# choice17/ransac_with_homography

Hardware: AMD Instinct MI355X
Metric: backward-warp Mpixels/sec (+ RANSAC hypotheses/sec) (higher is better)
Workload: dtype u8 (f64 coordinates, f32 blend); 1 GPU; transformImageH warp 3840x2160 RGB u8 bilinear -> 2028x3771 u8, 32 distinct frames per GPU per step, Hs mild perspective; full=False

## Files before the change

### ransac_with_homography_amd/csrc/rwh_warp_rgb8.h

```cpp
#pragma once
#include "rwh_common.h"
#include <type_traits>

namespace rwh {

typedef float f2 __attribute__((ext_vector_type(2)));

constexpr double MAGIC = 1572864.0;
constexpr uint32_t MAGIC_HI = 0x41380000u;
constexpr unsigned long long MAGIC_BITS = 0x4138000000000000ull;
constexpr float W_SCALE = 5.42101086242752217e-20f;
constexpr float U8_BIAS = -0.5f + 3.0517578125e-05f;

constexpr int FP_PX = 4;
constexpr int FP_ROWS = 9;
constexpr int FP_LANES = 21;
constexpr int FP_TEXELS = 4 * FP_LANES;
constexpr int FP_PITCH = 4 * FP_TEXELS + 16;

struct Coef {
    double cx[3], cy[3], cw[3];
    double dxs8[7][3];
    double ih[9];
    long long image;
// ... 840 lines not shown
            __builtin_amdgcn_fence(__ATOMIC_ACQUIRE, "wavefront");
        }
        const uint32_t bx = MAGIC_HI + (uint32_t)wxmn, by = MAGIC_HI + (uint32_t)wymn;
        const uint32_t rx_max = (uint32_t)(4 * wC - 2), ry_max = (uint32_t)(wnrows - 2);
#pragma unroll
        for (int h = 0; h < 2; ++h) {
            unsigned vbits = 0u;
            run_coords(h);
#pragma unroll
            for (int j = 0; j < FP_PX; ++j) {
                const bool valid = pixel_valid(j);
                weights2(lx[j], ly[j], valid ? WS : 0.f, valid ? WO : 0.f, valid ? WC : 0.f, wx0[j], wx1[j], wy0[j], wy1[j]);
                vbits |= (unsigned)valid << j;
                const uint32_t rx = min(hx[j] - bx, rx_max), ry = min(hy[j] - by, ry_max);
                const uint32_t lo = mad24_s(ry, (uint32_t)Win::LPITCH, rx << 2);
                const uint32_t* t0 = reinterpret_cast<const uint32_t*>(my + lo);
                const uint32_t* t1 = reinterpret_cast<const uint32_t*>(my + lo + Win::LPITCH);
                a0[j] = t0[0]; b0[j] = t0[1]; a1[j] = t1[0]; b1[j] = t1[1];
            }
            finish_masked_run(h, vbits);
        }
        return;
    }

    unsigned todo = 3u;
    if constexpr (HALVES) {
        todo = wpos ? 0u : 3u;
        if (wpos) {
            constexpr uint32_t lpitch = Win::LPITCH;
            chunk_t vh[2][Win::PASSES];
            int hrows[2];
            uint32_t tapc[2];
            bool hact[2];
#pragma unroll
            for (int h = 0; h < 2; ++h) {
                run_coords(h);
                const uint32_t lhx = h == 0 ? ehx[0] : hx[0], lhy = h == 0 ? ehy[0] : hy[0];
                const uint32_t rhx = h == 0 ? hx[3] : ehx[1], rhy = h == 0 ? hy[3] : ehy[1];
                const int hx0 = (int)__builtin_amdgcn_readlane(lhx, 0), hx1 = (int)__builtin_amdgcn_readlane(rhx, LPR - 1);
                const int hx2 = (int)__builtin_amdgcn_readlane(lhx, 64 - LPR), hx3 = (int)__builtin_amdgcn_readlane(rhx, 63);
                const int hy0 = (int)__builtin_amdgcn_readlane(lhy, 0), hy1 = (int)__builtin_amdgcn_readlane(rhy, LPR - 1);
                const int hy2 = (int)__builtin_amdgcn_readlane(lhy, 64 - LPR), hy3 = (int)__builtin_amdgcn_readlane(rhy, 63);
                const int qxmn = smin(smin(hx0, hx1), smin(hx2, hx3)) & ~3, qxmx = smax(smax(hx0, hx1), smax(hx2, hx3));
                const int qymn = smin(smin(hy0, hy1), smin(hy2, hy3)), qymx = smax(smax(hy0, hy1), smax(hy2, hy3));
                const int sxmn = (int)((uint32_t)smax(qxmn, 0) - MAGIC_HI), sxmx = (int)((uint32_t)smax(qxmx, 0) - MAGIC_HI);
                const int symn = (int)((uint32_t)smax(qymn, 0) - MAGIC_HI), symx = (int)((uint32_t)smax(qymx, 0) - MAGIC_HI);
                const int nr = symx - symn + 2, hC = (sxmx - sxmn + 5) >> 2;
                const bool hfits = (sxmn >= 0) & (sxmx < a.bound_w - 1) & (symn >= 0) & (symx < min(a.bound_h - 1, a.src_h - 2)) &
                                   (nr >= Win::RPP) & (nr <= Win::ROWS) & (hC <= Win::LPRW);
                hrows[h] = hfits ? nr : 0;
                hact[h] = (srow < Win::RPP) & (scol < hC);
                tapc[h] = ((uint32_t)qymn & 0xFFFFFFu) * lpitch + ((uint32_t)qxmn << 2) - slab_off_w;
                if (hfits) {
                    const unsigned char* gbase = simg + (size_t)((uint32_t)symn * pitch + (uint32_t)sxmn * (uint32_t)CH);
#pragma unroll
                    for (int p = 0; p < Win::PASSES; ++p)
                        if (p * Win::RPP < nr && hact[h])
                            __builtin_memcpy(&vh[h][p], gbase + (size_t)((uint32_t)min(p * Win::RPP, nr - Win::RPP) * pitch) + goff, sizeof(chunk_t));
                } else {
                    todo |= 1u << h;
                }
            }
#pragma unroll
            for (int h = 0; h < 2; ++h) {
                if (hrows[h] == 0) continue;
#pragma unroll
                for (int p = 0; p < Win::PASSES; ++p)
                    if (p * Win::RPP < hrows[h] && hact[h]) {
                        uint4 t4;
                        if constexpr (CH == 4) {
                            t4.x = vh[h][p].a; t4.y = vh[h][p].b; t4.z = vh[h][p].c; t4.w = vh[h][p].d;
                        } else {
                            t4.x = vh[h][p].a & 0xFFFFFFu;
                            t4.y = __builtin_amdgcn_perm(vh[h][p].b, vh[h][p].a, 0x0C050403u);
                            t4.z = __builtin_amdgcn_perm(vh[h][p].c, vh[h][p].b, 0x0C040302u);
                            t4.w = vh[h][p].c >> 8;
                        }
                        *reinterpret_cast<uint4*>(my + (uint32_t)min(p * Win::RPP, hrows[h] - Win::RPP) * lpitch + wl) = t4;
                    }
                __builtin_amdgcn_fence(__ATOMIC_RELEASE, "wavefront");
                __builtin_amdgcn_wave_barrier();
                __builtin_amdgcn_fence(__ATOMIC_ACQUIRE, "wavefront");
                if (h == 0) run_coords(0);
#pragma unroll
                for (int j = 0; j < FP_PX; ++j) {
                    weights2(lx[j], ly[j], WS, WO, WC, wx0[j], wx1[j], wy0[j], wy1[j]);
                    const uint32_t lo = mad24_s(hy[j], lpitch, shl2_add_s(hx[j], 0u - tapc[h]));
                    const uint32_t* t0 = reinterpret_cast<const uint32_t*>(slab0 + lo);
                    const uint32_t* t1 = reinterpret_cast<const uint32_t*>(slab0 + lo + lpitch);
                    a0[j] = t0[0]; b0[j] = t0[1]; a1[j] = t1[0]; b1[j] = t1[1];
                }
                const int first = tshift - (lcol + (PW / 2) * h);
                blend_store<DstT, PSTR, CH, true>(a0, b0, a1, b1, wx0, wx1, wy0, wy1, drow + CH * (PW / 2) * h,
                                                  store_any & (first <= 3 * PSTR), max(first, 0));
                __builtin_amdgcn_fence(__ATOMIC_RELEASE, "wavefront");
                __builtin_amdgcn_wave_barrier();
                if (h == 0 && hrows[1] != 0) run_coords(1);
            }
        }
        if (todo == 0u) return;
    }

#pragma unroll
    for (int h = 0; h < 2; ++h) {
        uint32_t off[FP_PX];
        bool near_end = false;
        unsigned vbits = 0u;
        if (HALVES && !(todo & (1u << h))) continue;
        run_coords(h);
#pragma unroll
        for (int j = 0; j < FP_PX; ++j) {
            const bool valid = pixel_valid(j);
            const int ix = (int)(hx[j] - MAGIC_HI), iy = (int)(hy[j] - MAGIC_HI);
            weights2(lx[j], ly[j], valid ? WS : 0.f, valid ? WO : 0.f, valid ? WC : 0.f, wx0[j], wx1[j], wy0[j], wy1[j]);
            off[j] = valid ? (uint32_t)iy * pitch + (uint32_t)ix * (uint32_t)CH : 0u;
            near_end |= valid & (iy > a.src_h - 3);
            vbits |= (unsigned)valid << j;
        }
        if (!__any(vbits != 0u)) {
#pragma unroll
            for (int j = 0; j < FP_PX; ++j) { a0[j] = 0u; b0[j] = 0u; a1[j] = 0u; b1[j] = 0u; }
        } else if (!__any(near_end)) {
#pragma unroll
            for (int j = 0; j < FP_PX; ++j) {
                const pk2 r0 = ld8(simg + off[j]);
                const pk2 r1 = ld8(simg + off[j] + pitch);
                if constexpr (CH == 4) { a0[j] = r0.a; b0[j] = r0.b; a1[j] = r1.a; b1[j] = r1.b; }
                else {
                    a0[j] = r0.a & 0xFFFFFFu; b0[j] = __builtin_amdgcn_perm(r0.b, r0.a, 0x0C050403u);
                    a1[j] = r1.a & 0xFFFFFFu; b1[j] = __builtin_amdgcn_perm(r1.b, r1.a, 0x0C050403u);
                }
            }
        } else {
            const uint32_t last = (uint32_t)a.src_h * pitch - (uint32_t)CH;
#pragma unroll
            for (int j = 0; j < FP_PX; ++j) {
                const uint32_t o00 = off[j];
                const uint32_t o01 = min(o00 + (uint32_t)CH, last), o10 = min(o00 + pitch, last), o11 = min(o00 + pitch + (uint32_t)CH, last);
                if constexpr (CH == 4) {
                    a0[j] = ld4(simg + o00); b0[j] = ld4(simg + o01); a1[j] = ld4(simg + o10); b1[j] = ld4(simg + o11);
                    continue;
                }
                a0[j] = simg[o00] | (simg[o00 + 1] << 8) | (simg[o00 + 2] << 16);
                b0[j] = simg[o01] | (simg[o01 + 1] << 8) | (simg[o01 + 2] << 16);
                a1[j] = simg[o10] | (simg[o10 + 1] << 8) | (simg[o10 + 2] << 16);
                b1[j] = simg[o11] | (simg[o11 + 1] << 8) | (simg[o11 + 2] << 16);
                if constexpr (EXT_SLAB) __builtin_amdgcn_sched_barrier(0);
            }
        }
        finish_masked_run(h, vbits);
    }
}

constexpr int F8_WALK_WAVES = 5;
template <int LOG_PW> __device__ __forceinline__ void fast8mb_body(const FastArgs& a);
template <typename DstT, int LOG_PW, bool WALK = false>
__global__ __launch_bounds__(256, (WALK ? F8_WALK_WAVES : f8_waves<DstT, LOG_PW>())) void warp_rgb8_fast8(const FastArgs a) {
    if constexpr (WALK) {
        static_assert(sizeof(DstT) == 1, "the batch form is uint8 in, uint8 out");
        fast8mb_body<LOG_PW>(a);
    } else {
        fast8_body<DstT, LOG_PW>(a, nullptr);
    }
}
#ifndef RWH_F8H_WAVES
#define RWH_F8H_WAVES(log_pw) ((log_pw) == 5 ? 4 : 5)
#endif
template <int LOG_PW>
__global__ __launch_bounds__(256, RWH_F8H_WAVES(LOG_PW)) void warp_rgb8_fast8h(const FastArgs a) { fast8_body<unsigned char, LOG_PW, false, 3, true>(a, nullptr); }
template <int LOG_PW>
__global__ __launch_bounds__(256, RWH_F8H_WAVES(LOG_PW)) void warp_rgb8_fast8h_tab(const FastArgs a, const CoefTab t) { fast8_body<unsigned char, LOG_PW, false, 3, true>(a, t.e); }
template <int LOG_PW>
__global__ __launch_bounds__(256, 6) void warp_rgba8_fast8(const FastArgs a) { fast8_body<unsigned char, LOG_PW, false, 4>(a, nullptr); }
template <int LOG_PW>
__global__ __launch_bounds__(256, 6) void warp_rgb8_comp(const FastArgs a, const CompArgs c) { fast8_body<unsigned char, LOG_PW, true>(a, nullptr, &c); }
template <typename DstT, int LOG_PW>
__global__ __launch_bounds__(256, (f8_waves<DstT, LOG_PW>())) void warp_rgb8_fast8_tab(const FastArgs a, const CoefTab t) { fast8_body<DstT, LOG_PW>(a, t.e); }

__device__ __forceinline__ pk3 pack_run_u8(const float (&o)[FP_PX][3]) {
    pk3 w;
    uint32_t q = 0;
    q = __builtin_amdgcn_cvt_pk_u8_f32(o[0][0], 0, q); q = __builtin_amdgcn_cvt_pk_u8_f32(o[0][1], 1, q);
    q = __builtin_amdgcn_cvt_pk_u8_f32(o[0][2], 2, q); q = __builtin_amdgcn_cvt_pk_u8_f32(o[1][0], 3, q);
    w.a = q; q = 0;
    q = __builtin_amdgcn_cvt_pk_u8_f32(o[1][1], 0, q); q = __builtin_amdgcn_cvt_pk_u8_f32(o[1][2], 1, q);
    q = __builtin_amdgcn_cvt_pk_u8_f32(o[2][0], 2, q); q = __builtin_amdgcn_cvt_pk_u8_f32(o[2][1], 3, q);
    w.b = q; q = 0;
    q = __builtin_amdgcn_cvt_pk_u8_f32(o[2][2], 0, q); q = __builtin_amdgcn_cvt_pk_u8_f32(o[3][0], 1, q);
    q = __builtin_amdgcn_cvt_pk_u8_f32(o[3][1], 2, q); q = __builtin_amdgcn_cvt_pk_u8_f32(o[3][2], 3, q);
    w.c = q;
    return w;
}
__device__ __forceinline__ void store_run_pk(const pk3& w, unsigned char* drow, bool store_any, int shift) {
    if (!store_any) return;
#ifdef RWH_F8M_STORE_MOD
    if (shift == 0) {
        typedef uint32_t u3s __attribute__((ext_vector_type(3)));
        const u3s d = {w.a, w.b, w.c};
        asm volatile("global_store_dwordx3 %0, %1, off " RWH_F8M_STORE_MOD "\n\ts_nop 2" : : "v"(drow), "v"(d) : "memory");
        return;
    }
#else
    if (shift == 0) { __builtin_memcpy(drow, &w, 12); return; }
#endif
    const unsigned long long lo8 = ((unsigned long long)w.b << 32) | w.a;
#pragma unroll
    for (int i = 3; i < 12; ++i)
        if (i >= 3 * shift) drow[i] = (unsigned char)(i < 8 ? lo8 >> (8 * i) : w.c >> (8 * (i - 8)));
}
#ifndef RWH_F8M_SKEW
#define RWH_F8M_SKEW 8
#endif
__device__ __forceinline__ void store_run_u8(const float (&o)[FP_PX][3], unsigned char* drow, bool store_any, int shift) {
    if (!store_any) return;
    if (shift == 0) {
        pk3 w;
        uint32_t q = 0;
        q = __builtin_amdgcn_cvt_pk_u8_f32(o[0][0], 0, q); q = __builtin_amdgcn_cvt_pk_u8_f32(o[0][1], 1, q);
        q = __builtin_amdgcn_cvt_pk_u8_f32(o[0][2], 2, q); q = __builtin_amdgcn_cvt_pk_u8_f32(o[1][0], 3, q);
        w.a = q; q = 0;
        q = __builtin_amdgcn_cvt_pk_u8_f32(o[1][1], 0, q); q = __builtin_amdgcn_cvt_pk_u8_f32(o[1][2], 1, q);
        q = __builtin_amdgcn_cvt_pk_u8_f32(o[2][0], 2, q); q = __builtin_amdgcn_cvt_pk_u8_f32(o[2][1], 3, q);
        w.b = q; q = 0;
        q = __builtin_amdgcn_cvt_pk_u8_f32(o[2][2], 0, q); q = __builtin_amdgcn_cvt_pk_u8_f32(o[3][0], 1, q);
        q = __builtin_amdgcn_cvt_pk_u8_f32(o[3][1], 2, q); q = __builtin_amdgcn_cvt_pk_u8_f32(o[3][2], 3, q);
        w.c = q;
        __builtin_memcpy(drow, &w, 12);
    } else {
#pragma unroll
        for (int j = 1; j < FP_PX; ++j)
            if (j >= shift) {
#pragma unroll
                for (int k = 0; k < 3; ++k) drow[3 * j + k] = (unsigned char)__builtin_amdgcn_cvt_pk_u8_f32(o[j][k], 0, 0);
            }
    }
}

template <int LOG_PW>
__device__ __forceinline__ void fast8m_body(const FastArgs& a) {
    constexpr int PW = 1 << LOG_PW, PH = 512 / PW, LPR = PW / 8, WX = 128 / PW;
    using Win = F8Window<LOG_PW>;
    constexpr uint32_t lpitch = Win::LPITCH + RWH_F8M_SKEW;
    constexpr int SLAB = ((Win::ROWS * (int)lpitch + 15) / 16) * 16;
    static_assert(SLAB >= Win::SLAB, "the per-frame fallback body shares this slab");
    constexpr float WS = W_SCALE * MIX_S, WO = W_ONE * MIX_S, WC = MIX_S;
    static_assert(MIX_RGB, "the multi-frame kernel is written for the float16-halves blend");
    unsigned char* const slab0 = wave_slabs<SLAB>();

    const unsigned b = blockIdx.x;
    const unsigned logical = (b & 7u) * a.mf_cpx + (b >> 3);
    if (logical >= a.mf_nblocks) return;
    const unsigned g = a.ntiles_magic ? __umulhi(logical, a.ntiles_magic) : (a.ntiles == 1u ? logical : 0u);
    const unsigned ti = logical - g * a.ntiles;
    const int f0 = (int)g * a.mf_frames, f1 = min(f0 + a.mf_frames, a.mf_batch);
    const unsigned ty = a.tiles_x_magic ? __umulhi(ti, a.tiles_x_magic) : ti;
    const unsigned tx = ti - ty * a.tiles_x;
    const int wave = __builtin_amdgcn_readfirstlane((int)(threadIdx.x >> 6));
    const int pwave = wave;
    {
        const int own_from = (int)tx * 128 - min((int)tx * 128, a.out_w - 128);
        if ((wave % WX + 1) * PW <= own_from) return;
    }
    const Coef& co = a.c;
    const int lane = threadIdx.x & 63;
    const int prow = lane / LPR, pq = lane % LPR;
    const int wave_x = (wave % WX) * PW, wave_y = (wave / WX) * PH;
    const int rr_raw = (int)ty * 16 + wave_y + prow;
    const int rr = min(rr_raw, a.rows - 1);
    const int tcol0 = (int)tx * 128;
    const int tcol = min(tcol0, a.out_w - 128);
    const int tshift = tcol0 - tcol;
    const int lcol = wave_x + pq * 4;
    const int c0p = tcol + lcol;
    const bool store_any = rr_raw < a.rows;
    const uint32_t pitch = (uint32_t)a.src_w * 3u;

    const double fr = (double)(a.row_begin + rr), fc = (double)c0p;
    const double X0 = fma(fc, co.cx[2], fma(fr, co.cx[1], co.cx[0]));
    const double Y0 = fma(fc, co.cy[2], fma(fr, co.cy[1], co.cy[0]));
    const double W0 = fma(fc, co.cw[2], fma(fr, co.cw[1], co.cw[0]));
    uint32_t ehx[2], ehy[2], elx[2], ely[2];
    bool wpos;
    {
        const double X7 = X0 + co.dxs8[6][0], Y7 = Y0 + co.dxs8[6][1], W7 = W0 + co.dxs8[6][2];
        double r0 = __builtin_amdgcn_rcp(W0); r0 = fma(fma(-W0, r0, 1.0), r0, r0);
        double r7 = __builtin_amdgcn_rcp(W7); r7 = fma(fma(-W7, r7, 1.0), r7, r7);
        const double ux0 = fma(X0, r0, MAGIC), uy0 = fma(Y0, r0, MAGIC), ux7 = fma(X7, r7, MAGIC), uy7 = fma(Y7, r7, MAGIC);
        ehx[0] = hi32(ux0); elx[0] = lo32(ux0); ehy[0] = hi32(uy0); ely[0] = lo32(uy0);
        ehx[1] = hi32(ux7); elx[1] = lo32(ux7); ehy[1] = hi32(uy7); ely[1] = lo32(uy7);
        const int h0 = (int)hi32(W0), h7 = (int)hi32(W7);
        wpos = __all((int)(h0 > 0x2D300000) & (int)(h0 < 0x52B00000) & (int)(h7 > 0x2D300000) & (int)(h7 < 0x52B00000));
    }
    const int x0 = (int)__builtin_amdgcn_readlane(ehx[0], 0), x1 = (int)__builtin_amdgcn_readlane(ehx[1], LPR - 1);
    const int x2 = (int)__builtin_amdgcn_readlane(ehx[0], 64 - LPR), x3 = (int)__builtin_amdgcn_readlane(ehx[1], 63);
    const int y0 = (int)__builtin_amdgcn_readlane(ehy[0], 0), y1 = (int)__builtin_amdgcn_readlane(ehy[1], LPR - 1);
    const int y2 = (int)__builtin_amdgcn_readlane(ehy[0], 64 - LPR), y3 = (int)__builtin_amdgcn_readlane(ehy[1], 63);
    const int hxmn = smin(smin(x0, x1), smin(x2, x3)) & ~3, hxmx = smax(smax(x0, x1), smax(x2, x3));
    const int hymn = smin(smin(y0, y1), smin(y2, y3)), hymx = smax(smax(y0, y1), smax(y2, y3));
    const int xmn = (int)((uint32_t)smax(hxmn, 0) - MAGIC_HI), xmx = (int)((uint32_t)smax(hxmx, 0) - MAGIC_HI);
    const int ymn = (int)((uint32_t)smax(hymn, 0) - MAGIC_HI), ymx = (int)((uint32_t)smax(hymx, 0) - MAGIC_HI);
    const int nrows = ymx - ymn + 2, C = (xmx - xmn + 5) >> 2;
    const bool staged = wpos & (xmn >= 0) & (xmx < a.bound_w - 1) & (ymn >= 0) & (ymx < min(a.bound_h - 1, a.src_h - 2)) &
                        (nrows >= Win::RPP) & (nrows <= Win::ROWS) & (C <= Win::LPRW);
    if (!staged) {
        for (int f = f0; f < f1; ++f)
            fast8_body<unsigned char, LOG_PW, false, 3, false, true>(a, nullptr, nullptr, (int)((unsigned)f * a.ntiles + ti), slab0 + pwave * SLAB);
        return;
// ... 26 lines not shown
#else
            asm volatile("s_mov_b64 %1, exec\n\ts_mov_b64 exec, %4\n\tglobal_load_dwordx3 %0, %2, %3\n\ts_mov_b64 exec, %1"
                         : "=&v"(v[p]), "=&s"(keep) : "v"(goff), "s"(rowbase), "s"(m) : "memory");
#endif
#endif
        }
    };
    auto landed = [&](u3 (&v)[Win::PASSES]) __attribute__((always_inline)) {
        if constexpr (Win::PASSES == 5) asm volatile("s_waitcnt vmcnt(0)" : "+v"(v[0]), "+v"(v[1]), "+v"(v[2]), "+v"(v[3]), "+v"(v[4]) : : "memory");
        else {
#pragma unroll
            for (int p = 0; p < Win::PASSES; ++p) asm volatile("s_waitcnt vmcnt(0)" : "+v"(v[p]) : : "memory");
        }
    };
    auto expand = [&](const u3 (&v)[Win::PASSES]) __attribute__((always_inline)) {
#pragma unroll
        for (int p = 0; p < Win::PASSES; ++p)
            if (p * Win::RPP < nrows && sactive) {
                const int r0 = min(p * Win::RPP, nrows - Win::RPP);
                uint4 t4;
                t4.x = v[p].x & 0xFFFFFFu;
                t4.y = __builtin_amdgcn_perm(v[p].y, v[p].x, 0x0C050403u);
                t4.z = __builtin_amdgcn_perm(v[p].z, v[p].y, 0x0C040302u);
                t4.w = v[p].z >> 8;
                __builtin_memcpy(__builtin_assume_aligned(my + (uint32_t)r0 * lpitch + wl, RWH_F8M_SKEW % 16 ? 8 : 16), &t4, 16);
            }
        __builtin_amdgcn_fence(__ATOMIC_RELEASE, "wavefront");
        __builtin_amdgcn_wave_barrier();
        __builtin_amdgcn_fence(__ATOMIC_ACQUIRE, "wavefront");
    };
    u3 v[Win::PASSES], v1[Win::PASSES];
#ifdef RWH_F8M_EARLY1
    issue(gsrc, v1);
#ifdef RWH_F8M_EARLY2
    if (f0 + 1 < f1) issue(gsrc + a.src_img_stride, v);
#endif
#endif

    const uint32_t slab_off = (uint32_t)pwave * (uint32_t)SLAB;
    const uint32_t tap_c = ((uint32_t)hymn & 0xFFFFFFu) * lpitch + ((uint32_t)hxmn << 2) - slab_off;
    float wa[F8_PX], wb[F8_PX], wc[F8_PX], wd[F8_PX];
    uint32_t lo[F8_PX];
#pragma unroll
    for (int h = 0; h < 2; ++h) {
        double X[3], Y[3], W[3], rc[3];
        uint32_t lx[FP_PX], ly[FP_PX], hx[FP_PX], hy[FP_PX];
#pragma unroll
        for (int j = 0; j < 3; ++j) { X[j] = X0 + co.dxs8[3 * h + j][0]; Y[j] = Y0 + co.dxs8[3 * h + j][1]; W[j] = W0 + co.dxs8[3 * h + j][2]; }
        const double p12 = W[0] * W[1], P = p12 * W[2];
        double rp = __builtin_amdgcn_rcp(P);
        rp = fma(fma(-P, rp, 1.0), rp, rp);
        const double r12 = rp * W[2];
        rc[2] = rp * p12; rc[0] = r12 * W[1]; rc[1] = r12 * W[0];
#pragma unroll
        for (int j = 0; j < 3; ++j) {
            const double ux = fma(X[j], rc[j], MAGIC), uy = fma(Y[j], rc[j], MAGIC);
            const int q = j + 1 - h;
            hx[q] = hi32(ux); lx[q] = lo32(ux); hy[q] = hi32(uy); ly[q] = lo32(uy);
        }
        hx[3 * h] = ehx[h]; lx[3 * h] = elx[h]; hy[3 * h] = ehy[h]; ly[3 * h] = ely[h];
#pragma unroll
        for (int j = 0; j < FP_PX; ++j) {
            const int p = 4 * h + j;
            const float wx1 = (float)lx[j], wy1 = (float)ly[j] * WS;
            const float w11 = wx1 * wy1;
            const float w01 = __builtin_fmaf(wx1, WO, -w11);
            const float w10 = __builtin_fmaf(wy1, 4294967296.0f, -w11);
            const float w00 = __builtin_fmaf(-wx1, WO, WC) - w10;
            wa[p] = w00; wb[p] = w01; wc[p] = w10; wd[p] = w11;
            lo[p] = mad24_s(hy[j], lpitch, shl2_add_s(hx[j], 0u - tap_c));
        }
    }

#ifdef RWH_F8M_EARLY1
#pragma unroll
    for (int p = 0; p < F8_PX; ++p) asm volatile("" : : "v"(wa[p]), "v"(wb[p]), "v"(wc[p]), "v"(wd[p]), "v"(lo[p]));
#else
    issue(gsrc, v1);
#endif
    landed(v1);
    expand(v1);
#ifndef RWH_F8M_EARLY2
    if (f0 + 1 < f1) issue(gsrc + a.src_img_stride, v);
#endif
#ifdef RWH_LAB_STAMPS
    unsigned long long tA = 0, tB = 0, tC = 0, tD = 0, t0 = __builtin_amdgcn_s_memtime(), t1;
#define RWH_STAMP(acc) { t1 = __builtin_amdgcn_s_memtime(); acc += t1 - t0; t0 = t1; }
#else
#define RWH_STAMP(acc)
#endif
    for (int f = f0; f < f1; ++f) {
        gsrc += a.src_img_stride;
        const bool more = f + 1 < f1;
        pk3 w[2];
#pragma unroll
        for (int h = 0; h < 2; ++h) {
            float o[FP_PX][3];
#pragma unroll
            for (int j = 0; j < FP_PX; ++j) {
                const int p = 4 * h + j;
                const uint32_t* t0 = reinterpret_cast<const uint32_t*>(slab0 + lo[p]);
                const uint32_t* t1 = reinterpret_cast<const uint32_t*>(slab0 + lo[p] + lpitch);
                const uint32_t a0 = t0[0], b0 = t0[1], a1 = t1[0], b1 = t1[1];
                const float w00 = wa[p], w01 = wb[p], w10 = wc[p], w11 = wd[p];
                const uint32_t g00 = rg_halves(a0), g01 = rg_halves(b0), g10 = rg_halves(a1), g11 = rg_halves(b1);
                o[j][0] = fmix_lo(g11, w11, fmix_lo(g10, w10, fmix_lo(g01, w01, fmix_lo_c(g00, w00, U8_BIAS))));
                o[j][1] = fmix_hi(g11, w11, fmix_hi(g10, w10, fmix_hi(g01, w01, fmix_hi_c(g00, w00, U8_BIAS))));
                o[j][2] = fmix_hi(b1, w11, fmix_hi(a1, w10, fmix_hi(b0, w01, fmix_hi_c(a0, w00, U8_BIAS))));
            }
            w[h] = pack_run_u8(o);
        }
        __builtin_amdgcn_fence(__ATOMIC_RELEASE, "wavefront");
        __builtin_amdgcn_wave_barrier();
        RWH_STAMP(tA)
        if (more) { landed(v); RWH_STAMP(tB) expand(v); }
        RWH_STAMP(tC)
        unsigned char* drow = gdst + doff;
#pragma unroll
        for (int h = 0; h < 2; ++h) {
            const int first = tshift - (lcol + (PW / 2) * h);
#ifdef RWH_ABL_M_NOSTORE
            if (w[h].a + w[h].b == 0x12345u)
#endif
            store_run_pk(w[h], drow + 3 * (PW / 2) * h, store_any & (first <= 3), max(first, 0));
        }
        gdst += a.dst_img_stride;
        if (f + 2 < f1) issue(gsrc + a.src_img_stride, v);
        RWH_STAMP(tD)
    }
#ifdef RWH_LAB_STAMPS
    if (lane == 0 && logical < 8192u) {
        unsigned long long* st = reinterpret_cast<unsigned long long*>(a.dst) + ((size_t)logical * 4 + pwave) * 4;
        st[0] = tA; st[1] = tB; st[2] = tC; st[3] = tD;
    }
#endif
}
constexpr int BCH = 36, BROWS = 21;
__device__ __forceinline__ void lds_barrier() { asm volatile("s_waitcnt lgkmcnt(0)\n\ts_barrier" : : : "memory"); }
__device__ __forceinline__ const FastArgs& kernarg_fastargs() {
    typedef const FastArgs __attribute__((address_space(4))) kFastArgs;
    kFastArgs* p = (kFastArgs*)__builtin_amdgcn_kernarg_segment_ptr();
    asm volatile("" : "+s"(p));
    return *(const FastArgs*)p;
}
template <int LOG_PW>
__device__ __forceinline__ void fast8mb_body(const FastArgs& a) {
    constexpr int PW = 1 << LOG_PW, PH = 512 / PW, LPR = PW / 8, WX = 128 / PW;
    using Win = F8Window<LOG_PW>;
    constexpr uint32_t lpitch = BCH * 16 + RWH_F8M_SKEW;
    constexpr int SLABW = ((Win::ROWS * (int)(Win::LPITCH + RWH_F8M_SKEW) + 15) / 16) * 16;
    static_assert(4 * SLABW >= BROWS * (int)lpitch + 128, "the block window lives in the four waves' slabs");
    constexpr float WS = W_SCALE * MIX_S, WO = W_ONE * MIX_S, WC = MIX_S;
    unsigned char* const slab0 = wave_slabs<SLABW>();

    const unsigned b = blockIdx.x;
    const unsigned logical = (b & 7u) * a.mf_cpx + (b >> 3);
    if (logical >= a.mf_nblocks) return;
    const unsigned g = a.ntiles_magic ? __umulhi(logical, a.ntiles_magic) : (a.ntiles == 1u ? logical : 0u);
    const unsigned ti = logical - g * a.ntiles;
    const int f0 = (int)g * a.mf_frames, f1 = min(f0 + a.mf_frames, a.mf_batch);
    const unsigned ty = a.tiles_x_magic ? __umulhi(ti, a.tiles_x_magic) : ti;
    const unsigned tx = ti - ty * a.tiles_x;
    const int wave = __builtin_amdgcn_readfirstlane((int)(threadIdx.x >> 6));
    const Coef& co = a.c;
    const int lane = threadIdx.x & 63;
    const int prow = lane / LPR, pq = lane % LPR;
    const int wave_x = (wave % WX) * PW, wave_y = (wave / WX) * PH;
    const int rr_raw = (int)ty * 16 + wave_y + prow;
    const int rr = min(rr_raw, a.rows - 1);
    const int tcol0 = (int)tx * 128;
    const int tcol = min(tcol0, a.out_w - 128);
    const int tshift = tcol0 - tcol;
    const int lcol = wave_x + pq * 4;
    const int c0p = tcol + lcol;
    const bool store_any = rr_raw < a.rows;
    const uint32_t pitch = (uint32_t)a.src_w * 3u;

    const double fr = (double)(a.row_begin + rr), fc = (double)c0p;
    const double X0 = fma(fc, co.cx[2], fma(fr, co.cx[1], co.cx[0]));
    const double Y0 = fma(fc, co.cy[2], fma(fr, co.cy[1], co.cy[0]));
    const double W0 = fma(fc, co.cw[2], fma(fr, co.cw[1], co.cw[0]));
    uint32_t ehx[2], ehy[2], elx[2], ely[2];
    bool wpos;
    {
        const double X7 = X0 + co.dxs8[6][0], Y7 = Y0 + co.dxs8[6][1], W7 = W0 + co.dxs8[6][2];
        double r0 = __builtin_amdgcn_rcp(W0); r0 = fma(fma(-W0, r0, 1.0), r0, r0);
        double r7 = __builtin_amdgcn_rcp(W7); r7 = fma(fma(-W7, r7, 1.0), r7, r7);
        const double ux0 = fma(X0, r0, MAGIC), uy0 = fma(Y0, r0, MAGIC), ux7 = fma(X7, r7, MAGIC), uy7 = fma(Y7, r7, MAGIC);
        ehx[0] = hi32(ux0); elx[0] = lo32(ux0); ehy[0] = hi32(uy0); ely[0] = lo32(uy0);
        ehx[1] = hi32(ux7); elx[1] = lo32(ux7); ehy[1] = hi32(uy7); ely[1] = lo32(uy7);
        const int h0 = (int)hi32(W0), h7 = (int)hi32(W7);
        wpos = __all((int)(h0 > 0x2D300000) & (int)(h0 < 0x52B00000) & (int)(h7 > 0x2D300000) & (int)(h7 < 0x52B00000));
    }
    const int x0 = (int)__builtin_amdgcn_readlane(ehx[0], 0), x1 = (int)__builtin_amdgcn_readlane(ehx[1], LPR - 1);
    const int x2 = (int)__builtin_amdgcn_readlane(ehx[0], 64 - LPR), x3 = (int)__builtin_amdgcn_readlane(ehx[1], 63);
    const int y0 = (int)__builtin_amdgcn_readlane(ehy[0], 0), y1 = (int)__builtin_amdgcn_readlane(ehy[1], LPR - 1);
    const int y2 = (int)__builtin_amdgcn_readlane(ehy[0], 64 - LPR), y3 = (int)__builtin_amdgcn_readlane(ehy[1], 63);
    const int whxmn = smin(smin(x0, x1), smin(x2, x3)) & ~3, whxmx = smax(smax(x0, x1), smax(x2, x3));
    const int whymn = smin(smin(y0, y1), smin(y2, y3)), whymx = smax(smax(y0, y1), smax(y2, y3));
    const bool owns = (wave % WX + 1) * PW > tshift;
    bool in;
    {
        const int bxmn = (int)((uint32_t)smax(whxmn, 0) - MAGIC_HI), bxmx = (int)((uint32_t)smax(whxmx, 0) - MAGIC_HI);
        const int bymn = (int)((uint32_t)smax(whymn, 0) - MAGIC_HI), bymx = (int)((uint32_t)smax(whymx, 0) - MAGIC_HI);
        const bool outside = wpos & ((bxmx < 0) | (bxmn >= a.bound_w) | (bymx < 0) | (bymn >= a.bound_h));
        const bool interior = wpos & (bxmn >= 0) & (bxmx < a.bound_w - 1) & (bymn >= 0) & (bymx < min(a.bound_h - 1, a.src_h - 2));
        in = owns & !outside;
        const int bw1 = __builtin_amdgcn_readfirstlane(a.bound_w) - 1, bh1 = __builtin_amdgcn_readfirstlane(a.bound_h) - 1;
        int* red = reinterpret_cast<int*>(slab0);
        if (lane == 0) {
            red[5 * wave] = in ? smin(smax(bxmn, 0), bw1) : 0x7FFFFFFF; red[5 * wave + 1] = in ? smin(smax(bxmx, 0), bw1) : -0x7FFFFFFF - 1;
            red[5 * wave + 2] = in ? smin(smax(bymn, 0), bh1) : 0x7FFFFFFF; red[5 * wave + 3] = in ? smin(smax(bymx, 0), bh1) : -0x7FFFFFFF - 1;
            red[5 * wave + 4] = (wpos ? 1 : 0) | ((interior | !owns) ? 2 : 0);
        }
    }
    __syncthreads();
    int xmn, xmx, ymn, ymx, fl_and;
    {
        const int* red = reinterpret_cast<const int*>(slab0);
        xmn = min(min(red[0], red[5]), min(red[10], red[15])); xmx = max(max(red[1], red[6]), max(red[11], red[16]));
        ymn = min(min(red[2], red[7]), min(red[12], red[17])); ymx = max(max(red[3], red[8]), max(red[13], red[18]));
        fl_and = red[4] & red[9] & red[14] & red[19];
        xmn = __builtin_amdgcn_readfirstlane(xmn) & ~3; xmx = __builtin_amdgcn_readfirstlane(xmx);
        ymn = __builtin_amdgcn_readfirstlane(ymn); ymx = __builtin_amdgcn_readfirstlane(ymx);
        fl_and = __builtin_amdgcn_readfirstlane(fl_and);
    }
    __syncthreads();
    const bool any_in = ymn != 0x7FFFFFFF;
    const int nrows = any_in ? ymx - ymn + 2 : 0, C = any_in ? (xmx - xmn + 5) >> 2 : 0;
    const uint32_t doff = ((uint32_t)rr * (uint32_t)a.pitch_w + (uint32_t)c0p) * 3u;
    const bool masked = !(fl_and & 2);
    if (!(fl_and & 1) || (any_in && !(nrows <= BROWS && C <= BCH && ymn + nrows - 1 <= a.src_h - 2))) {
        if (!owns) return;
        for (int f = f0; f < f1; ++f) {
            const FastArgs& ka = kernarg_fastargs();
            fast8_body<unsigned char, LOG_PW, false, 3, false, true>(ka, nullptr, nullptr, (int)((unsigned)f * ka.ntiles + ti), slab0 + wave * SLABW);
        }
        return;
    }
    if (!any_in) {
        if (!owns) return;
        unsigned char* drow = a.dst + (long long)f0 * a.dst_img_stride + doff;
        for (int f = f0; f < f1; ++f) {
#pragma unroll
            for (int h = 0; h < 2; ++h) {
                const int first = tshift - (lcol + (PW / 2) * h);
                zero_store<unsigned char, 1, 3>(drow + 3 * (PW / 2) * h, store_any & (first <= 3), max(first, 0));
            }
            drow += a.dst_img_stride;
        }
        return;
    }

    constexpr int SLOTS = (BROWS * BCH + 255) / 256;
    uint32_t goff[SLOTS], wl[SLOTS];
    unsigned long long smask[SLOTS];
    bool sact[SLOTS];
#pragma unroll
    for (int p = 0; p < SLOTS; ++p) {
        const int c = (int)threadIdx.x + 256 * p, r = c / BCH, k = c - r * BCH;
        sact[p] = (r < nrows) & (k < C);
        goff[p] = mad24_s((uint32_t)r, pitch, mul24_12((uint32_t)k));
        wl[p] = (uint32_t)r * lpitch + (uint32_t)k * 16u;
        smask[p] = __ballot(sact[p]);
    }
    const unsigned char* gsrc = a.src + (long long)f0 * a.src_img_stride + (size_t)((uint32_t)ymn * pitch + (uint32_t)xmn * 3u);
    unsigned char* gdst = a.dst + (long long)f0 * a.dst_img_stride;
    typedef uint32_t u3 __attribute__((ext_vector_type(3)));
    auto issue = [&](const unsigned char* gb, u3 (&v)[SLOTS]) __attribute__((always_inline)) {
#pragma unroll
        for (int p = 0; p < SLOTS; ++p) {
            unsigned long long keep;
            asm volatile("s_mov_b64 %1, exec\n\ts_mov_b64 exec, %4\n\tglobal_load_dwordx3 %0, %2, %3\n\ts_mov_b64 exec, %1"
                         : "=&v"(v[p]), "=&s"(keep) : "v"(goff[p]), "s"(gb), "s"(smask[p]) : "memory");
        }
    };
    auto landed = [&](u3 (&v)[SLOTS]) __attribute__((always_inline)) {
        static_assert(SLOTS == 3, "operand list below");
        asm volatile("s_waitcnt vmcnt(0)" : "+v"(v[0]), "+v"(v[1]), "+v"(v[2]) : : "memory");
    };
    auto expand = [&](const u3 (&v)[SLOTS]) __attribute__((always_inline)) {
#pragma unroll
        for (int p = 0; p < SLOTS; ++p)
            if (sact[p]) {
                uint4 t4;
                t4.x = v[p].x & 0xFFFFFFu;
                t4.y = __builtin_amdgcn_perm(v[p].y, v[p].x, 0x0C050403u);
                t4.z = __builtin_amdgcn_perm(v[p].z, v[p].y, 0x0C040302u);
                t4.w = v[p].z >> 8;
                __builtin_memcpy(__builtin_assume_aligned(slab0 + wl[p], RWH_F8M_SKEW % 16 ? 8 : 16), &t4, 16);
            }
    };

    const uint32_t bx = MAGIC_HI + (uint32_t)xmn, by = MAGIC_HI + (uint32_t)ymn;
    const uint32_t rx_max = (uint32_t)(4 * C - 2), ry_max = (uint32_t)(nrows - 2);
    const uint32_t tap_c = (by & 0xFFFFFFu) * lpitch + (bx << 2);
    float wa[F8_PX], wb[F8_PX], wc[F8_PX], wd[F8_PX];
    uint32_t lo[F8_PX];
    u3 v[SLOTS];
    issue(gsrc, v);
    if (in) {
#pragma unroll
    for (int h = 0; h < 2; ++h) {
        double X[3], Y[3], W[3], rc[3];
        uint32_t lx[FP_PX], ly[FP_PX], hx[FP_PX], hy[FP_PX];
#pragma unroll
        for (int j = 0; j < 3; ++j) { X[j] = X0 + co.dxs8[3 * h + j][0]; Y[j] = Y0 + co.dxs8[3 * h + j][1]; W[j] = W0 + co.dxs8[3 * h + j][2]; }
        const double p12 = W[0] * W[1], P = p12 * W[2];
        double rp = __builtin_amdgcn_rcp(P);
        rp = fma(fma(-P, rp, 1.0), rp, rp);
        const double r12 = rp * W[2];
        rc[2] = rp * p12; rc[0] = r12 * W[1]; rc[1] = r12 * W[0];
#pragma unroll
        for (int j = 0; j < 3; ++j) {
            const double ux = fma(X[j], rc[j], MAGIC), uy = fma(Y[j], rc[j], MAGIC);
            const int q = j + 1 - h;
            hx[q] = hi32(ux); lx[q] = lo32(ux); hy[q] = hi32(uy); ly[q] = lo32(uy);
        }
        hx[3 * h] = ehx[h]; lx[3 * h] = elx[h]; hy[3 * h] = ehy[h]; ly[3 * h] = ely[h];
        if (!masked) {
#pragma unroll
            for (int j = 0; j < FP_PX; ++j) {
                const int p = 4 * h + j;
                const float wx1 = (float)lx[j], wy1 = (float)ly[j] * WS;
                const float w11 = wx1 * wy1;
                const float w01 = __builtin_fmaf(wx1, WO, -w11);
                const float w10 = __builtin_fmaf(wy1, 4294967296.0f, -w11);
                const float w00 = __builtin_fmaf(-wx1, WO, WC) - w10;
                wa[p] = w00; wb[p] = w01; wc[p] = w10; wd[p] = w11;
                lo[p] = mad24_s(hy[j], lpitch, shl2_add_s(hx[j], 0u - tap_c));
            }
        } else {
#pragma unroll
            for (int j = 0; j < FP_PX; ++j) {
                const int p = 4 * h + j;
                const unsigned long long ubx = ((unsigned long long)hx[j] << 32) | lx[j], uby = ((unsigned long long)hy[j] << 32) | ly[j];
                const bool valid = (ubx >= MAGIC_BITS) & (ubx <= a.xmax_bits) & (uby >= MAGIC_BITS) & (uby <= a.ymax_bits);
                const float ws = valid ? WS : 0.f, wo = valid ? WO : 0.f, wc1 = valid ? WC : 0.f;
                const float wx1 = (float)lx[j], wy1 = (float)ly[j] * ws;
                const float w11 = wx1 * wy1;
                const float w01 = __builtin_fmaf(wx1, wo, -w11);
                const float w10 = __builtin_fmaf(wy1, 4294967296.0f, -w11);
                const float w00 = __builtin_fmaf(-wx1, wo, wc1) - w10;
                wa[p] = w00; wb[p] = w01; wc[p] = w10; wd[p] = w11;
                const uint32_t rx = min(hx[j] - bx, rx_max), ry = min(hy[j] - by, ry_max);
                lo[p] = mad24_s(ry, lpitch, rx << 2);
            }
        }
    }
    }
    landed(v);
    expand(v);
    lds_barrier();
    if (f0 + 1 < f1) issue(gsrc + a.src_img_stride, v);
    for (int f = f0; f < f1; ++f) {
        gsrc += a.src_img_stride;
        const bool more = f + 1 < f1;
        pk3 w[2];
        if (in) {
#pragma unroll
        for (int h = 0; h < 2; ++h) {
            float o[FP_PX][3];
#pragma unroll
            for (int j = 0; j < FP_PX; ++j) {
                const int p = 4 * h + j;
                const uint32_t* t0 = reinterpret_cast<const uint32_t*>(slab0 + lo[p]);
                const uint32_t* t1 = reinterpret_cast<const uint32_t*>(slab0 + lo[p] + lpitch);
                const uint32_t a0 = t0[0], b0 = t0[1], a1 = t1[0], b1 = t1[1];
                const float w00 = wa[p], w01 = wb[p], w10 = wc[p], w11 = wd[p];
                const uint32_t g00 = rg_halves(a0), g01 = rg_halves(b0), g10 = rg_halves(a1), g11 = rg_halves(b1);
                o[j][0] = fmix_lo(g11, w11, fmix_lo(g10, w10, fmix_lo(g01, w01, fmix_lo_c(g00, w00, U8_BIAS))));
                o[j][1] = fmix_hi(g11, w11, fmix_hi(g10, w10, fmix_hi(g01, w01, fmix_hi_c(g00, w00, U8_BIAS))));
                o[j][2] = fmix_hi(b1, w11, fmix_hi(a1, w10, fmix_hi(b0, w01, fmix_hi_c(a0, w00, U8_BIAS))));
            }
            w[h] = pack_run_u8(o);
        }
        }
        if (more) {
            lds_barrier();
            landed(v);
            expand(v);
            lds_barrier();
        }
        unsigned char* drow = gdst + doff;
        if (in) {
#pragma unroll
            for (int h = 0; h < 2; ++h) {
                const int first = tshift - (lcol + (PW / 2) * h);
                store_run_pk(w[h], drow + 3 * (PW / 2) * h, store_any & (first <= 3), max(first, 0));
            }
        } else if (owns) {
#pragma unroll
            for (int h = 0; h < 2; ++h) {
                const int first = tshift - (lcol + (PW / 2) * h);
                zero_store<unsigned char, 1, 3>(drow + 3 * (PW / 2) * h, store_any & (first <= 3), max(first, 0));
            }
        }
        gdst += a.dst_img_stride;
        if (f + 2 < f1) issue(gsrc + a.src_img_stride, v);
    }
}
template <int LOG_PW>
__global__ __launch_bounds__(256, 4) void warp_rgb8_fast8mb(const FastArgs a) { fast8mb_body<LOG_PW>(a); }

#ifndef RWH_F8M_WAVES
#define RWH_F8M_WAVES 4
#endif
template <int LOG_PW>
__global__ __launch_bounds__(256, RWH_F8M_WAVES) void warp_rgb8_fast8m(const FastArgs a) { fast8m_body<LOG_PW>(a); }

#ifndef RWH_STRIP_MAX
#define RWH_STRIP_MAX 16
#endif
constexpr int STRIP_MAX = RWH_STRIP_MAX;
template <typename DstT>
__device__ __forceinline__ void strip_body(const FastArgs& a, const Coef* tab) {
    constexpr bool U8 = sizeof(DstT) == 1;
    constexpr float WS = W_SCALE * MIX_S, WO = W_ONE * MIX_S, WC = MIX_S, BIAS = U8 ? U8_BIAS : 0.f;
    const int rr = (int)(blockIdx.x * 256 + threadIdx.x);
    const unsigned img = blockIdx.y;
    if (rr >= a.rows) return;
    const Coef& co = tab ? tab[img] : a.c;
    const unsigned img_mem = tab ? (unsigned)co.image : img;
    const unsigned char* simg = a.src + (long long)img_mem * a.src_img_stride;
    DstT* drow = reinterpret_cast<DstT*>(a.dst + (long long)img_mem * a.dst_img_stride) + ((size_t)rr * (size_t)a.pitch_w) * 3;
    const uint32_t pitch = (uint32_t)a.src_w * 3u, last = (uint32_t)a.src_h * pitch - 3u;
    const double fr = (double)(a.row_begin + rr);
    for (int c = a.out_w; c < a.pitch_w; ++c) {
        const double fc = (double)c;
        const double X = fma(fc, co.cx[2], fma(fr, co.cx[1], co.cx[0]));
        const double Y = fma(fc, co.cy[2], fma(fr, co.cy[1], co.cy[0]));
        const double W = fma(fc, co.cw[2], fma(fr, co.cw[1], co.cw[0]));
        double r = __builtin_amdgcn_rcp(W);
        r = fma(fma(-W, r, 1.0), r, r);
        const double ux = fma(X, r, MAGIC), uy = fma(Y, r, MAGIC);
        const unsigned long long ubx = (unsigned long long)__double_as_longlong(ux), uby = (unsigned long long)__double_as_longlong(uy);
        const bool valid = (ubx >= MAGIC_BITS) & (ubx <= a.xmax_bits) & (uby >= MAGIC_BITS) & (uby <= a.ymax_bits);
        float o[3] = {BIAS, BIAS, BIAS};
        if (valid) {
            const int ix = (int)(hi32(ux) - MAGIC_HI), iy = (int)(hi32(uy) - MAGIC_HI);
            const float wx1 = (float)lo32(ux), wy1 = (float)lo32(uy) * WS;
            const float w11 = wx1 * wy1;
            const float w01 = __builtin_fmaf(wx1, WO, -w11);
            const float w10 = __builtin_fmaf(wy1, 4294967296.0f, -w11);
            const float w00 = __builtin_fmaf(-wx1, WO, WC) - w10;
            const uint32_t o00 = (uint32_t)iy * pitch + (uint32_t)ix * 3u;
            const uint32_t o01 = min(o00 + 3u, last), o10 = min(o00 + pitch, last), o11 = min(o00 + pitch + 3u, last);
#pragma unroll
            for (int k = 0; k < 3; ++k) {
                const float p00 = (float)simg[o00 + k] * 0x1p-24f, p01 = (float)simg[o01 + k] * 0x1p-24f;
                const float p10 = (float)simg[o10 + k] * 0x1p-24f, p11 = (float)simg[o11 + k] * 0x1p-24f;
                o[k] = __builtin_fmaf(p11, w11, __builtin_fmaf(p10, w10, __builtin_fmaf(p01, w01, __builtin_fmaf(p00, w00, BIAS))));
            }
        }
#pragma unroll
        for (int k = 0; k < 3; ++k) {
            if constexpr (U8) drow[3 * c + k] = (unsigned char)__builtin_amdgcn_cvt_pk_u8_f32(o[k], 0, 0);
            else drow[3 * c + k] = o[k];
        }
    }
}
template <typename DstT>
__global__ __launch_bounds__(256) void warp_rgb8_strip(const FastArgs a) { strip_body<DstT>(a, nullptr); }
template <typename DstT>
__global__ __launch_bounds__(256) void warp_rgb8_strip_tab(const FastArgs a, const CoefTab t) { strip_body<DstT>(a, t.e); }

constexpr uint32_t NN_TIE = 1u << 12;

__device__ __forceinline__ uint32_t nn_exact_texel(const FastArgs& a, const double (&ih)[9], const unsigned char* simg, int r, int c) {
    const double x = (c == a.out_w - 1) ? a.gx_last : (double)c * a.gstep_x + a.gx0;
    const double y = (r == a.out_h - 1) ? a.gy_last : (double)r * a.gstep_y + a.gy0;
    const double X = fma(ih[1], y, ih[0] * x) + ih[2];
    const double Y = fma(ih[4], y, ih[3] * x) + ih[5];
    const double W = fma(ih[7], y, ih[6] * x) + ih[8];
    const double sx = X / W, sy = Y / W;
    const int xi = (int)(sx + 0.5), yi = (int)(sy + 0.5);
    if (!((xi >= 0) & (xi <= a.bound_w - 1) & (yi >= 0) & (yi <= a.bound_h - 1) & (sx == sx) & (sy == sy))) return 0u;
    const uint32_t off = ((uint32_t)yi * (uint32_t)a.src_w + (uint32_t)xi) * 3u;
    const uint32_t img_bytes = (uint32_t)a.src_h * (uint32_t)a.src_w * 3u;
    if (off + 4u <= img_bytes) return ld4(simg + off) & 0xFFFFFFu;
    return simg[off] | (simg[off + 1] << 8) | (simg[off + 2] << 16);
}

__device__ __forceinline__ void nn_store(const uint32_t (&t)[FP_PX], unsigned char* drow, bool store_any, int first) {
    if (!store_any) return;
    if (first <= 0) {
        pk3 w;
        w.a = (t[0] & 0xFFFFFFu) | (t[1] << 24);
        w.b = ((t[1] >> 8) & 0xFFFFu) | (t[2] << 16);
        w.c = ((t[2] >> 16) & 0xFFu) | (t[3] << 8);
        __builtin_memcpy(drow, &w, 12);
    } else {
#pragma unroll
        for (int j = 1; j < FP_PX; ++j)
            if (j >= first) { drow[3 * j] = (unsigned char)t[j]; drow[3 * j + 1] = (unsigned char)(t[j] >> 8); drow[3 * j + 2] = (unsigned char)(t[j] >> 16); }
    }
}

template <int LOG_PW>
__device__ __forceinline__ void nn_body(const FastArgs& a, const Coef* tab) {
    constexpr int PW = 1 << LOG_PW, PH = 512 / PW, LPR = PW / 8, WX = 128 / PW;
    constexpr double MAGIC_R = MAGIC + 0.5;
    __shared__ __attribute__((aligned(16))) unsigned char slab[4][F8Window<LOG_PW>::SLAB];

    const unsigned b = blockIdx.x;
    const unsigned logical = (b & 7u) * a.cpx + (b >> 3);
    if (logical >= a.nblocks) return;
    const unsigned t = a.tiles_x_magic ? __umulhi(logical, a.tiles_x_magic) : logical;
    const unsigned tx = logical - t * a.tiles_x;
    const unsigned img = a.tiles_y_magic ? __umulhi(t, a.tiles_y_magic) : t;
    const unsigned ty = t - img * a.tiles_y;
    const Coef& co = tab ? tab[img] : a.c;
    const unsigned img_mem = tab ? (unsigned)co.image : img;
    double ih9[9];
#pragma unroll
    for (int i = 0; i < 9; ++i) ih9[i] = co.ih[i];
    const int wave = __builtin_amdgcn_readfirstlane((int)(threadIdx.x >> 6));
    const int lane = threadIdx.x & 63;
    const int prow = lane / LPR, pq = lane % LPR;
    const int wave_x = (wave % WX) * PW, wave_y = (wave / WX) * PH;
    const int rr_raw = (int)ty * 16 + wave_y + prow;
    const int rr = min(rr_raw, a.rows - 1);
    const int tcol0 = (int)tx * 128, tcol = min(tcol0, a.out_w - 128), tshift = tcol0 - tcol;
    if ((wave_x + PW <= tshift) | ((int)ty * 16 + wave_y >= a.rows)) return;
    const int lcol = wave_x + pq * 4, c0p = tcol + lcol;
    const bool store_any = rr_raw < a.rows;
    const unsigned char* simg = a.src + (long long)img_mem * a.src_img_stride;
    unsigned char* drow = a.dst + (long long)img_mem * a.dst_img_stride + ((uint32_t)rr * (uint32_t)a.pitch_w + (uint32_t)c0p) * 3u;
    const uint32_t pitch = (uint32_t)a.src_w * 3u;
    const int out_row = a.row_begin + rr;

    const double fr = (double)out_row, fc = (double)c0p;
    const double X0 = fma(fc, co.cx[2], fma(fr, co.cx[1], co.cx[0]));
    const double Y0 = fma(fc, co.cy[2], fma(fr, co.cy[1], co.cy[0]));
    const double W0 = fma(fc, co.cw[2], fma(fr, co.cw[1], co.cw[0]));
    uint32_t ehx[2], ehy[2], elx[2], ely[2];
    bool wpos;
    {
        const double X7 = X0 + co.dxs8[6][0], Y7 = Y0 + co.dxs8[6][1], W7 = W0 + co.dxs8[6][2];
        double r0 = __builtin_amdgcn_rcp(W0); r0 = fma(fma(-W0, r0, 1.0), r0, r0);
        double r7 = __builtin_amdgcn_rcp(W7); r7 = fma(fma(-W7, r7, 1.0), r7, r7);
        const double ux0 = fma(X0, r0, MAGIC_R), uy0 = fma(Y0, r0, MAGIC_R), ux7 = fma(X7, r7, MAGIC_R), uy7 = fma(Y7, r7, MAGIC_R);
        ehx[0] = hi32(ux0); elx[0] = lo32(ux0); ehy[0] = hi32(uy0); ely[0] = lo32(uy0);
        ehx[1] = hi32(ux7); elx[1] = lo32(ux7); ehy[1] = hi32(uy7); ely[1] = lo32(uy7);
        const int h0 = (int)hi32(W0), h7 = (int)hi32(W7);
        wpos = __all((int)(h0 > 0x2D300000) & (int)(h0 < 0x52B00000) & (int)(h7 > 0x2D300000) & (int)(h7 < 0x52B00000));
    }
    uint32_t lx[FP_PX], ly[FP_PX], hx[FP_PX], hy[FP_PX];
// ... 140 lines not shown
```

Baseline: 766,300 Mpix/s.

## Stage warped tile through LDS and store coalesced 16-byte rows; simplify staging slots

Output pixels are now written into an LDS tile image, and after a barrier the whole block copies that tile to global memory as contiguous 16-byte stores per row, instead of each lane storing its own scattered 12-byte runs. The source-window staging is restructured into three fixed slots of seven rows with one shared offset and a per-slot base pointer, which cuts register use. The walk kernel's launch-bounds wave target rises from 5 to 6. The aim is better write coalescing and lower VGPR pressure, paid for by an extra LDS barrier and round trip per frame, plus byte-wise stores at partially owned tile edges.

New measurement: 746,800 Mpix/s. 0.975x the previous value.

```diff
diff --git a/ransac_with_homography_amd/csrc/rwh_warp_rgb8.h b/ransac_with_homography_amd/csrc/rwh_warp_rgb8.h
--- a/ransac_with_homography_amd/csrc/rwh_warp_rgb8.h
+++ b/ransac_with_homography_amd/csrc/rwh_warp_rgb8.h
@@ -1016,7 +1016,7 @@
     }
 }
 
-constexpr int F8_WALK_WAVES = 5;
+constexpr int F8_WALK_WAVES = 6;
 template <int LOG_PW> __device__ __forceinline__ void fast8mb_body(const FastArgs& a);
 template <typename DstT, int LOG_PW, bool WALK = false>
 __global__ __launch_bounds__(256, (WALK ? F8_WALK_WAVES : f8_waves<DstT, LOG_PW>())) void warp_rgb8_fast8(const FastArgs a) {
@@ -1349,6 +1349,9 @@
     static_assert(4 * SLABW >= BROWS * (int)lpitch + 128, "the block window lives in the four waves' slabs");
     constexpr float WS = W_SCALE * MIX_S, WO = W_ONE * MIX_S, WC = MIX_S;
     unsigned char* const slab0 = wave_slabs<SLABW>();
+    constexpr int TILE_IMG = ((BROWS * (int)lpitch + 15) / 16) * 16;
+    static_assert(4 * SLABW - TILE_IMG >= 16 * 384, "the tile image lives behind the block window, inside the block's allocation");
+    unsigned char* const tile_img = slab0 + TILE_IMG;
 
     const unsigned b = blockIdx.x;
     const unsigned logical = (b & 7u) * a.mf_cpx + (b >> 3);
@@ -1370,7 +1373,6 @@
     const int tshift = tcol0 - tcol;
     const int lcol = wave_x + pq * 4;
     const int c0p = tcol + lcol;
-    const bool store_any = rr_raw < a.rows;
     const uint32_t pitch = (uint32_t)a.src_w * 3u;
 
     const double fr = (double)(a.row_begin + rr), fc = (double)c0p;
@@ -1425,7 +1427,6 @@
     __syncthreads();
     const bool any_in = ymn != 0x7FFFFFFF;
     const int nrows = any_in ? ymx - ymn + 2 : 0, C = any_in ? (xmx - xmn + 5) >> 2 : 0;
-    const uint32_t doff = ((uint32_t)rr * (uint32_t)a.pitch_w + (uint32_t)c0p) * 3u;
     const bool masked = !(fl_and & 2);
     if (!(fl_and & 1) || (any_in && !(nrows <= BROWS && C <= BCH && ymn + nrows - 1 <= a.src_h - 2))) {
         if (!owns) return;
@@ -1437,30 +1438,37 @@
     }
     if (!any_in) {
         if (!owns) return;
-        unsigned char* drow = a.dst + (long long)f0 * a.dst_img_stride + doff;
+        uint32_t t = threadIdx.x;
+        asm volatile("" : "+v"(t));
+        const int zrow = (int)ty * 16 + wave_y + (int)(t & 63u) / LPR, zcol = wave_x + (int)(t & 63u) % LPR * 4;
+        unsigned char* drow = a.dst + (long long)f0 * a.dst_img_stride + ((uint32_t)min(zrow, a.rows - 1) * (uint32_t)a.pitch_w + (uint32_t)(tcol + zcol)) * 3u;
         for (int f = f0; f < f1; ++f) {
 #pragma unroll
             for (int h = 0; h < 2; ++h) {
-                const int first = tshift - (lcol + (PW / 2) * h);
-                zero_store<unsigned char, 1, 3>(drow + 3 * (PW / 2) * h, store_any & (first <= 3), max(first, 0));
+                const int first = tshift - (zcol + (PW / 2) * h);
+                zero_store<unsigned char, 1, 3>(drow + 3 * (PW / 2) * h, (zrow < a.rows) & (first <= 3), max(first, 0));
             }
             drow += a.dst_img_stride;
         }
         return;
     }
 
-    constexpr int SLOTS = (BROWS * BCH + 255) / 256;
-    uint32_t goff[SLOTS], wl[SLOTS];
+    static_assert(BROWS == 21, "three staging slots of seven window rows");
+    constexpr int SLOTS = 3, SROWS = BROWS / SLOTS;
+    const int sr = (int)threadIdx.x / BCH, sk = (int)threadIdx.x - sr * BCH;
+    const uint32_t goff = mad24_s((uint32_t)sr, pitch, mul24_12((uint32_t)sk));
+    static_assert(lpitch % 8 == 0, "window rows start on multiples of 8 bytes");
+    uint32_t wl8 = (uint32_t)sr * (lpitch / 8) + (uint32_t)sk * 2u;
+    asm volatile("" : "+v"(wl8));
     unsigned long long smask[SLOTS];
     bool sact[SLOTS];
+    const int srow = ((sr < SROWS) & (sk < C)) ? sr : 0x7FFF;
 #pragma unroll
     for (int p = 0; p < SLOTS; ++p) {
-        const int c = (int)threadIdx.x + 256 * p, r = c / BCH, k = c - r * BCH;
-        sact[p] = (r < nrows) & (k < C);
-        goff[p] = mad24_s((uint32_t)r, pitch, mul24_12((uint32_t)k));
-        wl[p] = (uint32_t)r * lpitch + (uint32_t)k * 16u;
-        smask[p] = __ballot(sact[p]);
-    }
+        sact[p] = srow < nrows - SROWS * p;
+        smask[p] = __builtin_amdgcn_ballot_w64(sact[p]);
+    }
+    const uint32_t spitch = (uint32_t)SROWS * pitch;
     const unsigned char* gsrc = a.src + (long long)f0 * a.src_img_stride + (size_t)((uint32_t)ymn * pitch + (uint32_t)xmn * 3u);
     unsigned char* gdst = a.dst + (long long)f0 * a.dst_img_stride;
     typedef uint32_t u3 __attribute__((ext_vector_type(3)));
@@ -1469,7 +1477,7 @@
         for (int p = 0; p < SLOTS; ++p) {
             unsigned long long keep;
             asm volatile("s_mov_b64 %1, exec\n\ts_mov_b64 exec, %4\n\tglobal_load_dwordx3 %0, %2, %3\n\ts_mov_b64 exec, %1"
-                         : "=&v"(v[p]), "=&s"(keep) : "v"(goff[p]), "s"(gb), "s"(smask[p]) : "memory");
+                         : "=&v"(v[p]), "=&s"(keep) : "v"(goff), "s"(gb + (size_t)p * spitch), "s"(smask[p]) : "memory");
         }
     };
     auto landed = [&](u3 (&v)[SLOTS]) __attribute__((always_inline)) {
@@ -1485,7 +1493,9 @@
                 t4.y = __builtin_amdgcn_perm(v[p].y, v[p].x, 0x0C050403u);
                 t4.z = __builtin_amdgcn_perm(v[p].z, v[p].y, 0x0C040302u);
                 t4.w = v[p].z >> 8;
-                __builtin_memcpy(__builtin_assume_aligned(slab0 + wl[p], RWH_F8M_SKEW % 16 ? 8 : 16), &t4, 16);
+                uint32_t ws = wl8 + (uint32_t)(SROWS * p) * (lpitch / 8);
+                asm volatile("" : "+v"(ws));
+                __builtin_memcpy(__builtin_assume_aligned(slab0 + (ws << 3), RWH_F8M_SKEW % 16 ? 8 : 16), &t4, 16);
             }
     };
 
@@ -1573,24 +1583,47 @@
             w[h] = pack_run_u8(o);
         }
         }
+        lds_barrier();
+        if (owns) {
+            uint32_t* const rrun = reinterpret_cast<uint32_t*>(tile_img + (uint32_t)(wave_y + prow) * 384u + (uint32_t)lcol * 3u);
+#pragma unroll
+            for (int h = 0; h < 2; ++h) {
+                uint32_t* const q = rrun + 3 * (PW / 2) / 4 * h;
+                q[0] = in ? w[h].a : 0u; q[1] = in ? w[h].b : 0u; q[2] = in ? w[h].c : 0u;
+            }
+        }
         if (more) {
-            lds_barrier();
             landed(v);
             expand(v);
-            lds_barrier();
-        }
-        unsigned char* drow = gdst + doff;
-        if (in) {
-#pragma unroll
-            for (int h = 0; h < 2; ++h) {
-                const int first = tshift - (lcol + (PW / 2) * h);
-                store_run_pk(w[h], drow + 3 * (PW / 2) * h, store_any & (first <= 3), max(first, 0));
-            }
-        } else if (owns) {
-#pragma unroll
-            for (int h = 0; h < 2; ++h) {
-                const int first = tshift - (lcol + (PW / 2) * h);
-                zero_store<unsigned char, 1, 3>(drow + 3 * (PW / 2) * h, store_any & (first <= 3), max(first, 0));
+        }
+        lds_barrier();
+        {
+            uint32_t t = threadIdx.x;
+            asm volatile("" : "+v"(t));
+            unsigned char* const dtile = gdst + ((uint32_t)ty * 16u * (uint32_t)a.pitch_w + (uint32_t)tcol) * 3u;
+            const int own_b = 3 * tshift;
+#pragma unroll
+            for (int ps = 0; ps < 2; ++ps) {
+                const uint32_t q = t + 256u * ps, prw = q / 24u, kb = (q - prw * 24u) * 16u;
+                const int cut = own_b - (int)kb;
+                if ((ps == 0 || q < 384u) & ((int)(ty * 16u + prw) < a.rows) & (cut < 16)) {
+                    const uint4 d = *reinterpret_cast<const uint4*>(tile_img + q * 16u);
+                    unsigned char* const dp = dtile + (prw * (uint32_t)a.pitch_w * 3u + kb);
+                    if (cut <= 0) {
+#ifdef RWH_F8M_STORE_MOD
+                        typedef uint32_t u4s __attribute__((ext_vector_type(4)));
+                        const u4s dv = {d.x, d.y, d.z, d.w};
+                        asm volatile("global_store_dwordx4 %0, %1, off " RWH_F8M_STORE_MOD "\n\ts_nop 2" : : "v"(dp), "v"(dv) : "memory");
+#else
+                        __builtin_memcpy(dp, &d, 16);
+#endif
+                    } else {
+                        const uint32_t dw[4] = {d.x, d.y, d.z, d.w};
+#pragma unroll
+                        for (int i = 1; i < 16; ++i)
+                            if (i >= cut) dp[i] = (unsigned char)(dw[i / 4] >> (8 * (i % 4)));
+                    }
+                }
             }
         }
         gdst += a.dst_img_stride;
```
